# zhuker/lamejs

Measured on NVIDIA H100. Metric: encoded audio seconds/sec (44.1kHz stereo 128kbps CBR), higher is better.
Workload: dtype f64

## Files before the change

### lamejs_b200/csrc/k_quant.cuh

```cuda
#ifndef MP3B200_K_QUANT_CUH
#define MP3B200_K_QUANT_CUH
#include <stddef.h>
#include "mp3_device.cuh"
#include "mp3_tables.h"
#include "k_psy.cuh"

#define Q_LARGE_BITS 100000
#define Q_IXMAX 8206
#define Q_FULL 0xffffffffu

struct GranuleInfoDev {
  int global_gain, part2_3_length, part2_length, big_values, count1, scalefac_compress;
  int table_select[3], region0_count, region1_count, preflag, scalefac_scale, count1table_select, block_type;
  int subblock_gain[4];
  int count1bits, sfbmax, sfbdivide, sfb_lmax, psymax, psy_lmax, sfb_smin, max_nonzero_coeff;
  int scalefac[MP3_SFBMAX];
  int slen[4];
  int part_row;
  int pad_;
  double xrpow_max;
};
struct QuantFrameState {
  int stream, rel_frame;
  int in_old[2], in_step[2];
// ... 21 lines not shown
__device__ int g_t33l[16];
__constant__ int c_slen1_n[16];
__constant__ int c_slen2_n[16];
__device__ int g_slen_n[2][16];
__device__ int g_scale_tab[2][16];
__device__ unsigned int g_cat_tab[8][256];
__constant__ int c_slen1_tab[16];
__constant__ int c_slen2_tab[16];
__constant__ int c_huf_noesc[15];

static int quant_upload_constants() {
  static const int t32l[16] = {1, 5, 5, 7, 5, 8, 7, 9, 5, 7, 7, 9, 7, 9, 9, 10};
  static const int t33l[16] = {4, 5, 5, 6, 5, 6, 6, 7, 5, 6, 6, 7, 6, 7, 7, 8};
  static const int s1n[16] = {1, 1, 1, 1, 8, 2, 2, 2, 4, 4, 4, 8, 8, 8, 16, 16};
  static const int s2n[16] = {1, 2, 4, 8, 1, 2, 4, 8, 2, 4, 8, 2, 4, 8, 4, 8};
  static const int s1t[16] = {0, 0, 0, 0, 3, 1, 1, 1, 2, 2, 2, 3, 3, 3, 4, 4};
  static const int s2t[16] = {0, 1, 2, 3, 0, 1, 2, 3, 1, 2, 3, 1, 2, 3, 2, 3};
  static const int ss[16] = {0, 18, 36, 54, 54, 36, 54, 72, 54, 72, 90, 72, 90, 108, 108, 126};
  static const int sl[16] = {0, 10, 20, 30, 33, 21, 31, 41, 32, 42, 52, 43, 53, 63, 64, 74};
  static const int hn[15] = {1, 2, 5, 7, 7, 10, 10, 13, 13, 13, 13, 13, 13, 13, 13};
#define UP(sym, src) if (cudaMemcpyToSymbol(sym, src, sizeof(src)) != cudaSuccess) return -100
  UP(g_huff_code, MP3_HUFF_CODE); UP(g_huff_len, MP3_HUFF_LEN); UP(c_huff_off, MP3_HUFF_OFF);
  UP(c_huff_xlen, MP3_HUFF_XLEN);
  UP(g_t32l, t32l); UP(g_t33l, t33l); UP(c_slen1_n, s1n); UP(c_slen2_n, s2n);
  UP(c_slen1_tab, s1t); UP(c_slen2_tab, s2t); UP(c_huf_noesc, hn);
  {
    static int sn[2][16], st[2][16];
    static unsigned int ct[8][256];
    for (int k = 0; k < 16; k++) { sn[0][k] = s1n[k]; sn[1][k] = s2n[k]; st[0][k] = sl[k]; st[1][k] = ss[k]; }
    static const int fam[6] = {1, 2, 5, 7, 10, 13};
    for (int x = 0; x < 16; x++) for (int y = 0; y < 16; y++) {
      const int q = x * 16 + y;
      for (int c = 0; c < 6; c++) {
        const int t1 = fam[c], xl = MP3_HUFF_XLEN[t1];
        unsigned a = 0, b = 0, d = 0;
        if (x < xl && y < xl) {
          const int i = x * xl + y;
          if (c == 0) a = b = d = MP3_HUFF_LEN[MP3_HUFF_OFF[1] + i];
          else if (c == 1) { a = MP3_HUFF_TABLE23[i] >> 16; b = d = MP3_HUFF_TABLE23[i] & 0xffff; }
          else if (c == 2) { a = MP3_HUFF_TABLE56[i] >> 16; b = d = MP3_HUFF_TABLE56[i] & 0xffff; }
          else { a = MP3_HUFF_LEN[MP3_HUFF_OFF[t1] + i]; b = MP3_HUFF_LEN[MP3_HUFF_OFF[t1 + 1] + i]; d = MP3_HUFF_LEN[MP3_HUFF_OFF[t1 + 2] + i]; }
        }
        ct[c][q] = a | (b << 11) | (d << 22);
      }
      { const unsigned a = MP3_HUFF_LARGETBL[q] >> 16, b = MP3_HUFF_LARGETBL[q] & 0xffff; ct[6][q] = a | (b << 11) | (b << 22); }
      ct[7][q] = 0;
    }
    UP(g_slen_n, sn); UP(g_scale_tab, st); UP(g_cat_tab, ct);
  }
#undef UP
  return 0;
}

struct __align__(16) GcWork {
  float xrpow[576];
  short ixw[576];
  short* ixg;
  GranuleInfoDev w, b;
  const Mp3Geo* geo;
  float xmin[MP3_SFBMAX], distort[MP3_SFBMAX];
  int pn_step[MP3_SFBMAX]; float pn_noise[MP3_SFBMAX], pn_noise_log[MP3_SFBMAX];
  int pn_global_gain, pn_sfb_count1;
  unsigned char mode[MP3_SFBMAX + 1];
  short nstart[MP3_SFBMAX], nlen[MP3_SFBMAX];
  int scratch[8];
  double dscratch[4];
  __align__(16) float xr[576];
};
struct __align__(16) WarpShared {
  double ath[6];
  int scfsi[4];
  GcWork wk;
};
#define Q_STRIDE_NOXR ((int)((offsetof(WarpShared, wk) + offsetof(GcWork, xr) + 15) & ~(size_t)15))
static_assert((offsetof(WarpShared, wk) + offsetof(GcWork, xr)) % 16 == 0 && (offsetof(WarpShared, wk) + offsetof(GcWork, xrpow)) % 16 == 0 &&
              (offsetof(WarpShared, wk) + offsetof(GcWork, ixw)) % 16 == 0 && sizeof(WarpShared) % 16 == 0, "rows are moved as 16-byte vectors");
#ifndef Q_SLIM_BLOCKS
#define Q_SLIM_BLOCKS 9
#endif

#define LANE (threadIdx.x & 31)
#ifdef Q_TASKSTAT
__device__ int g_taskstat[1 << 16][8];
#endif
#ifdef Q_STATS
__device__ unsigned long long g_qstats[16];
#define QSTAT(i) do { if (LANE == 0) atomicAdd(&g_qstats[i], 1ull); } while (0)
#else
#define QSTAT(i) do { } while (0)
#endif
#define Q_PRAGMA(x) _Pragma(#x)
#define Q_UNROLL(n) Q_PRAGMA(unroll n)
#ifndef Q_RT_UNROLL
#define Q_RT_UNROLL 1
#endif
#ifndef Q_CB_UNROLL
#define Q_CB_UNROLL 1
#endif
#ifndef Q_CN_UNROLL
#define Q_CN_UNROLL 2
#endif
#ifndef Q_HELPER
#define Q_HELPER __forceinline__
#endif
#ifndef Q_SPEC_START
#define Q_SPEC_START 180
#endif
#ifndef Q_SPEC_STEP
#define Q_SPEC_STEP 32
#endif
#ifndef Q_SPEC_GR1_STEP
#define Q_SPEC_GR1_STEP 2
#endif
#ifndef Q_SPEC_FOLD
#define Q_SPEC_FOLD 1
#endif
#ifndef Q_MIN_BLOCKS
#define Q_MIN_BLOCKS 14
#endif
__device__ __noinline__ double q_log10(double x) { return m3_log10(x); }
__device__ __noinline__ double q_pow(double x, double y) { return m3_pow(x, y); }
__device__ __forceinline__ int wmax(int v) { return __reduce_max_sync(Q_FULL, v); }
__device__ __forceinline__ int wsum(int v) { return __reduce_add_sync(Q_FULL, v); }
__device__ __forceinline__ unsigned wsumu(unsigned v) { return __reduce_add_sync(Q_FULL, v); }

struct RegionClass { int cat; unsigned lin; int t1, t2; };
__device__ Q_HELPER RegionClass region_class(int mx) {
  RegionClass rc;
  rc.lin = 0; rc.t2 = 0;
  if (mx == 0) { rc.cat = 7; rc.t1 = 0; }
  else if (mx <= 15) {
    rc.t1 = c_huf_noesc[mx - 1];
    rc.cat = mx <= 3 ? mx - 1 : (mx <= 5 ? 3 : (mx <= 7 ? 4 : 5));
  } else {
    const int n = 32 - __clz(mx - 15);
    rc.t2 = 24 + (int)((0x7777665432100000ull >> (4 * n)) & 15ull);
    rc.t1 = max(rc.t2 - 8, 16 + (int)((0x7777766554432100ull >> (4 * n)) & 15ull));
    const unsigned la = (unsigned)c_huff_xlen[rc.t1], lb = (unsigned)c_huff_xlen[rc.t2];
    rc.lin = la | (lb << 11) | (lb << 22);
    rc.cat = 6;
  }
  return rc;
}
__device__ __forceinline__ unsigned pair_bits(unsigned w, int cat, unsigned lin) {
  const unsigned x = w & 0xffffu, y = w >> 16;
  const unsigned xe = min(x, 15u), ye = min(y, 15u);
  return __ldg(&g_cat_tab[cat][xe * 16 + ye]) + ((x > 14u) + (y > 14u)) * lin;
}
__device__ Q_HELPER int region_pick(int mx, const RegionClass& rc, int a, int b, int c, int* bits) {
  if (mx > Q_IXMAX) { *bits = Q_LARGE_BITS; return -1; }
  if (mx == 0) return 0;
  int t = rc.t1;
  if (mx <= 15) {
    if (a > b) { a = b; t++; }
    if (a > c) { a = c; t = rc.t1 + 2; }
  } else if (a > b) { a = b; t = rc.t2; }
  *bits += a;
  return t;
}

__device__ __noinline__ int region_table_w(const short* ix, int begin, int end, int* bits) {
  const int lane = LANE;
  const unsigned* w32 = reinterpret_cast<const unsigned*>(ix);
  const int p0 = (begin >> 1) + lane, p1 = end >> 1;
  unsigned m = 0;
Q_UNROLL(Q_RT_UNROLL)
// ... 275 lines not shown
  const bool is_short = gi->block_type == BT_SHORT;
  const int sfbmax = gi->sfbmax, sfbdivide = gi->sfbdivide;
  __syncwarp();
  if (!is_short && 0 == gi->preflag) {
    const bool in = lane >= 11 && lane < 21;
    const int pt = pretab_of(lane);
    const bool ok = !in || scalefac[lane] >= pt;
    if (__all_sync(Q_FULL, ok)) {
      __syncwarp();
      if (in) scalefac[lane] -= pt;
      if (lane == 0) gi->preflag = 1;
      __syncwarp();
    }
  }
  int m1 = 0, m2 = 0;
#pragma unroll 1
  for (int sfb = lane; sfb < sfbmax; sfb += 32) {
    const int v = scalefac[sfb];
    if (sfb < sfbdivide) m1 = max(m1, v); else m2 = max(m2, v);
  }
  m1 = wmax(m1); m2 = wmax(m2);
  int key = Q_LARGE_BITS * 16 + 15;
  if (lane < 16 && m1 < __ldg(&g_slen_n[0][lane]) && m2 < __ldg(&g_slen_n[1][lane])) key = __ldg(&g_scale_tab[is_short ? 1 : 0][lane]) * 16 + lane;
  key = __reduce_min_sync(Q_FULL, key);
  const int p2 = key >> 4;
  if (lane == 0) { gi->part2_length = p2; if (p2 != Q_LARGE_BITS) gi->scalefac_compress = key & 15; }
  __syncwarp();
  return p2 == Q_LARGE_BITS;
}

__device__ __noinline__ bool scale_bitcount_lsf_w(GranuleInfoDev* gi) {
  const int lane = LANE;
  const bool is_short = gi->block_type == BT_SHORT;
  __syncwarp();
  int m0 = 0, m1 = 0, m2 = 0, m3 = 0;
  const int n = is_short ? 36 : 21;
#pragma unroll 1
  for (int i = lane; i < n; i += 32) {
    const int v = gi->scalefac[i];
    const int p = is_short ? i / 9 : (i < 6 ? 0 : (i - 6) / 5 + 1);
    if (p == 0) m0 = max(m0, v); else if (p == 1) m1 = max(m1, v); else if (p == 2) m2 = max(m2, v); else m3 = max(m3, v);
  }
  m0 = wmax(m0); m1 = wmax(m1); m2 = wmax(m2); m3 = wmax(m3);
  const bool over = m0 > 15 || m1 > 15 || m2 > 7 || m3 > 7;
  if (!over && lane == 0) {
    const int s1 = m0 ? 32 - __clz(m0) : 0, s2 = m1 ? 32 - __clz(m1) : 0, s3 = m2 ? 32 - __clz(m2) : 0, s4 = m3 ? 32 - __clz(m3) : 0;
    gi->slen[0] = s1; gi->slen[1] = s2; gi->slen[2] = s3; gi->slen[3] = s4;
    gi->part_row = is_short ? 1 : 0;
    gi->scalefac_compress = (((s1 * 5) + s2) << 4) + (s3 << 2) + s4;
    gi->part2_length = is_short ? 9 * (s1 + s2 + s3 + s4) : 6 * s1 + 5 * (s2 + s3 + s4);
  }
  __syncwarp();
  return over;
}
__device__ __forceinline__ bool scale_bitcount_any_w(GranuleInfoDev* gi, int mode_gr) {
  return mode_gr == 2 ? scale_bitcount_w(gi) : scale_bitcount_lsf_w(gi);
}

__device__ __forceinline__ bool loop_break_w(const GranuleInfoDev* gi, const GcWork* wk) {
  bool nz = true;
#pragma unroll 1
  for (int sfb = LANE; sfb < gi->sfbmax; sfb += 32)
    if (gi->scalefac[sfb] + gi->subblock_gain[wk->geo->window[sfb]] == 0) nz = false;
  return __all_sync(Q_FULL, nz);
}

__device__ __noinline__ void scale_xrpow_w(GcWork* wk, GranuleInfoDev* gi, double f34) {
  const int lane = LANE;
  const int sfbmax = gi->sfbmax;
  float mx = 0.0f;
#pragma unroll 1
  for (int p = lane; p < 288; p += 32) {
    const int sfb = wk->geo->sfb_of_line[2 * p];
    if (sfb < sfbmax && wk->mode[sfb]) {
      float2* xp = reinterpret_cast<float2*>(&wk->xrpow[2 * p]);
      float2 x = *xp;
      f32s v0, v1; v0.v = x.x; v1.v = x.y;
      v0 *= f34; v1 *= f34;
      x.x = v0.v; x.y = v1.v;
      *xp = x;
      mx = fmaxf(mx, fmaxf(v0.v, v1.v));
    }
  }
#pragma unroll 1
  for (int o = 16; o > 0; o >>= 1) mx = fmaxf(mx, __shfl_xor_sync(Q_FULL, mx, o));
  if (lane == 0 && (double)mx > gi->xrpow_max) gi->xrpow_max = (double)mx;
  __syncwarp();
}

__device__ __noinline__ bool balance_escalate_w(const Mp3Tables* T, GcWork* wk) {
  const int lane = LANE;
  GranuleInfoDev* gi = &wk->w;
  int* flag = &wk->scratch[0];
  bool status = true;
  const int scale_now = gi->scalefac_scale, is_short_blk = gi->block_type == BT_SHORT;
  __syncwarp();
  if (T->noise_shaping > 1) {
    if (0 == scale_now) {
      {
        const int sfbmax = gi->sfbmax, pre = gi->preflag;
#pragma unroll 1
        for (int sfb = lane; sfb < sfbmax; sfb += 32) {
          int s = gi->scalefac[sfb];
          if (pre != 0) s += pretab_of(sfb);
          const int odd = (s & 1) != 0;
          if (odd) s++;
          wk->mode[sfb] = (unsigned char)odd;
          gi->scalefac[sfb] = s >> 1;
        }
        __syncwarp();
        if (lane == 0) { gi->preflag = 0; gi->scalefac_scale = 1; }
      }
      __syncwarp();
      scale_xrpow_w(wk, gi, 1.29683955465100964055);
      status = false;
    } else if (is_short_blk) {
      if (lane == 0) {
        int ret = 0;
        int* scalefac = gi->scalefac;
#pragma unroll 1
        for (int i = 0; i < MP3_SFBMAX; i++) wk->nlen[i] = -1;
#pragma unroll 1
        for (int window = 0; window < 3 && !ret; window++) {
          int s1 = 0, s2 = 0, sfb;
#pragma unroll 1
          for (sfb = gi->sfb_lmax + window; sfb < gi->sfbdivide; sfb += 3) if (s1 < scalefac[sfb]) s1 = scalefac[sfb];
#pragma unroll 1
          for (; sfb < gi->sfbmax; sfb += 3) if (s2 < scalefac[sfb]) s2 = scalefac[sfb];
          if (s1 < 16 && s2 < 8) continue;
          if (gi->subblock_gain[window] >= 7) { ret = 1; break; }
          gi->subblock_gain[window]++;
#pragma unroll 1
          for (sfb = gi->sfb_lmax + window; sfb < gi->sfbmax; sfb += 3) {
            int s = scalefac[sfb];
            s = s - (4 >> gi->scalefac_scale);
            if (s >= 0) { scalefac[sfb] = s; continue; }
            scalefac[sfb] = 0;
            wk->nlen[sfb] = 210 + s * (1 << (gi->scalefac_scale + 1));
          }
          wk->nlen[sfb] = 202;
        }
        *flag = ret;
      }
      __syncwarp();
      {
        float mx = 0.0f;
#pragma unroll 1
        for (int i = lane; i < 576; i += 32) {
          const int sfb = wk->geo->sfb_of_line[i];
          if (sfb < MP3_SFBMAX && wk->nlen[sfb] >= 0) {
            f32s v; v.v = wk->xrpow[i];
            v *= (double)T->ipow20[wk->nlen[sfb]];
            wk->xrpow[i] = v.v;
            mx = fmaxf(mx, v.v);
          }
        }
        for (int o = 16; o > 0; o >>= 1) mx = fmaxf(mx, __shfl_xor_sync(Q_FULL, mx, o));
        if (lane == 0 && (double)mx > gi->xrpow_max) gi->xrpow_max = (double)mx;
        __syncwarp();
      }
      {
        const int bailed = *flag;
        __syncwarp();
        status = bailed != 0 || loop_break_w(gi, wk);
      }
    }
  }
  if (!status) status = scale_bitcount_any_w(gi, T->mode_gr);
  return !status;
}


__device__ __noinline__ bool balance_noise_w(const Mp3Tables* T, GcWork* wk) {
  const int lane = LANE;
  GranuleInfoDev* gi = &wk->w;
  const double ifq = gi->scalefac_scale == 0 ? 1.29683955465100964055 : 1.68179283050742922612;
  {
    const int sfbmax = gi->sfbmax;
    double trigger = 0;
#pragma unroll 1
    for (int sfb = lane; sfb < sfbmax; sfb += 32) if (trigger < (double)wk->distort[sfb]) trigger = (double)wk->distort[sfb];
    for (int o = 16; o > 0; o >>= 1) { const double t = __shfl_xor_sync(Q_FULL, trigger, o); if (trigger < t) trigger = t; }
    if (trigger > 1.0) trigger = sqrt(trigger);
    else trigger *= .95;
#pragma unroll 1
    for (int sfb = lane; sfb < sfbmax; sfb += 32) {
      const int amp = !((double)wk->distort[sfb] < trigger);
      wk->mode[sfb] = (unsigned char)amp;
      if (amp) gi->scalefac[sfb]++;
    }
  }
  __syncwarp();
  scale_xrpow_w(wk, gi, ifq);
  int r;
  if (loop_break_w(gi, wk)) r = 0;
  else r = scale_bitcount_any_w(gi, T->mode_gr) ? 2 : 1;
  if (r == 0) return false;
  if (r == 1) return true;
  return balance_escalate_w(T, wk);
}

__device__ __noinline__ void copy_gi_w(GranuleInfoDev* dst, const GranuleInfoDev* src) {
  const int n = sizeof(GranuleInfoDev) / 4;
  const int* s = reinterpret_cast<const int*>(src);
  int* d = reinterpret_cast<int*>(dst);
  __syncwarp();
  static_assert(sizeof(GranuleInfoDev) / 4 <= 96, "three rounds");
  int v[3];
#pragma unroll
  for (int k = 0; k < 3; k++) { const int i = LANE + 32 * k; if (i < n) v[k] = s[i]; }
#pragma unroll
  for (int k = 0; k < 3; k++) { const int i = LANE + 32 * k; if (i < n) d[i] = v[k]; }
  __syncwarp();
}
__device__ __noinline__ void copy_ix_w(short* dst, const short* src) {
  const int* s = reinterpret_cast<const int*>(src);
  int* d = reinterpret_cast<int*>(dst);
  __syncwarp();
#pragma unroll 1
  for (int i = LANE; i < 288; i += 32) d[i] = s[i];
  __syncwarp();
}

__device__ __noinline__ int bin_search_w(const Mp3Tables* T, GcWork* wk, int desired_rate, int* old_value, int* current_step, int stat_base = 0) {
  GranuleInfoDev* gi = &wk->b;
  int nBits;
  int CurrentStep = *current_step;
  bool flagGoneOver = false;
  const int start = *old_value;
  int Direction = 0;
  int gain = start;
  desired_rate -= gi->part2_length;
  __syncwarp();
  for (;;) {
    int step;
    if (LANE == 0) gi->global_gain = gain;
    __syncwarp();
    QSTAT(stat_base);
    nBits = count_bits_w<false>(T, wk, gi, wk->ixw);
    if (CurrentStep == 1 || nBits == desired_rate) break;
    if (nBits > desired_rate) {
      if (Direction == 2) flagGoneOver = true;
      if (flagGoneOver) CurrentStep /= 2;
      Direction = 1;
      step = CurrentStep;
    } else {
      if (Direction == 1) flagGoneOver = true;
      if (flagGoneOver) CurrentStep /= 2;
      Direction = 2;
      step = -CurrentStep;
    }
    gain += step;
    if (gain < 0) { gain = 0; flagGoneOver = true; }
    if (gain > 255) { gain = 255; flagGoneOver = true; }
  }
  while (nBits > desired_rate && gain < 255) {
    gain++;
    if (LANE == 0) gi->global_gain = gain;
    __syncwarp();
    QSTAT(stat_base + 1);
    nBits = count_bits_w<false>(T, wk, gi, wk->ixw);
  }
  *current_step = (start - gain >= 4) ? 4 : 2;
  *old_value = gain;
  if (LANE == 0) gi->part2_3_length = nBits;
  __syncwarp();
  return nBits;
}

__device__ __noinline__ unsigned long long gi_hash(const GranuleInfoDev* gi) {
  const unsigned* w = reinterpret_cast<const unsigned*>(gi);
  unsigned sum = 0, x = 0;
#pragma unroll 1
  for (int i = LANE; i < (int)(sizeof(GranuleInfoDev) / 4); i += 32) {
    unsigned v = (w[i] ^ ((unsigned)i * 0x9E3779B9u)) * 0x85EBCA6Bu;
    v ^= v >> 13; v *= 0xC2B2AE35u; v ^= v >> 16;
    sum += v; x ^= __funnelshift_l(v, v, i & 31);
  }
  sum = __reduce_add_sync(Q_FULL, sum);
  x = __reduce_xor_sync(Q_FULL, x);
  return ((unsigned long long)sum << 32) | x;
}

__device__ __noinline__ void outer_loop_w(const Mp3Tables* T, GcWork* wk, int targ_bits) {
  const int lane = LANE;
  NoiseRes best, cur;
  int best_part2_3_length = 9999999;
#pragma unroll 1
  for (int i = lane; i < MP3_SFBMAX; i += 32) { wk->pn_step[i] = 0; wk->pn_noise[i] = 0.0f; wk->pn_noise_log[i] = 0.0f; }
  if (lane == 0) { wk->pn_global_gain = 0; wk->pn_sfb_count1 = 0; }
  __syncwarp();
  calc_noise_w(T, wk, &wk->b, wk->ixw, &best);
  best.bits = wk->b.part2_3_length;
  copy_gi_w(&wk->w, &wk->b);
  bool best_here = true;
  int age = 0;
  const int quant_comp = T->quant_comp;
  (void)quant_comp;
  do {
    const int search_limit = 3;
    int maxggain = 255;
    if (!balance_noise_w(T, wk)) break;
    GranuleInfoDev* w = &wk->w;
    if (w->scalefac_scale != 0) maxggain = 254;
    const int huff_bits = targ_bits - w->part2_length;
    if (huff_bits <= 0) break;
    int p23, gg;
    if (best_here) { copy_ix_w(wk->ixg, wk->ixw); best_here = false; }
    int sc_in;
    for (;;) {
      sc_in = wk->pn_sfb_count1;
      QSTAT(8);
      p23 = count_bits_w<true>(T, wk, w, wk->ixw);
      gg = w->global_gain;
      __syncwarp();
      if (!(p23 > huff_bits && gg <= maxggain)) break;
      if (lane == 0) w->global_gain = gg + 1;
      __syncwarp();
    }
    if (lane == 0) w->part2_3_length = p23;
    __syncwarp();
    if (gg > maxggain) break;
    if (best.over_count == 0) {
      bool repeat = wk->pn_sfb_count1 == sc_in;
      for (;;) {
        if (!repeat) { QSTAT(9); p23 = count_bits_w<true>(T, wk, w, wk->ixw); }
        repeat = false;
        gg = w->global_gain;
        __syncwarp();
        if (!(p23 > best_part2_3_length && gg <= maxggain)) break;
        if (lane == 0) w->global_gain = gg + 1;
        __syncwarp();
      }
      if (lane == 0) w->part2_3_length = p23;
      __syncwarp();
      if (gg > maxggain) break;
    }
    QSTAT(10);
    calc_noise_w(T, wk, w, wk->ixw, &cur);
    cur.bits = w->part2_3_length;
    bool better;
    if (best.over_count > 0) {
      better = cur.over_SSD <= best.over_SSD;
      if (cur.over_SSD == best.over_SSD) better = cur.bits < best.bits;
    } else {
      better = ((cur.max_noise < 0) && ((cur.max_noise * 10 + cur.bits) <= (best.max_noise * 10 + best.bits)));
    }
    if (best.over_count == 0) better = better && cur.bits < best.bits;
    if (better) {
      best_part2_3_length = wk->b.part2_3_length;
      best = cur;
      copy_gi_w(&wk->b, &wk->w);
      best_here = true;
      age = 0;
    } else {
      if (++age > search_limit && best.over_count == 0) break;
    }
    const int cont = (wk->w.global_gain + wk->w.scalefac_scale) < 255;
    __syncwarp();
    if (!cont) break;
  } while (true);
  if (!best_here) copy_ix_w(wk->ixw, wk->ixg);
}

__device__ __noinline__ double ath_adjust_dev(double a, double x, double athFloor) {
  const double o = 90.30873362, p = 94.82444863;
  double u = q_log10(x) * 10.0;
  const double v = a * a;
  double w = 0.0;
  u -= athFloor;
  if (v > 1E-20) w = 1. + q_log10(v) * (10.0 / o);
  if (w < 0) w = 0.;
  u *= w;
  u += athFloor + o - p;
  return q_pow(10., 0.1 * u);
}

__device__ __noinline__ bool gc_prepare_w(const Mp3Tables* T, GcWork* wk, const double* ath_ps, const float* __restrict__ xr_g, int block_type,
                             const PsyRatioDev* __restrict__ ratio, double ath_adjust) {
  const bool need_xmin = true;
  const int lane = LANE;
  GranuleInfoDev* gi = &wk->b;
  const bool is_short = block_type == BT_SHORT;
  if (lane == 0) {
    gi->part2_3_length = 0; gi->big_values = 0; gi->count1 = 0; gi->global_gain = 210; gi->scalefac_compress = 0;
    gi->table_select[0] = gi->table_select[1] = gi->table_select[2] = 0;
    gi->subblock_gain[0] = gi->subblock_gain[1] = gi->subblock_gain[2] = gi->subblock_gain[3] = 0;
    gi->region0_count = 0; gi->region1_count = 0; gi->preflag = 0; gi->scalefac_scale = 0; gi->count1table_select = 0;
    gi->part2_length = 0; gi->block_type = block_type; gi->count1bits = 0;
    gi->sfb_lmax = is_short ? 0 : 21; gi->sfb_smin = is_short ? 0 : 12;
    gi->psy_lmax = is_short ? 0 : 21;
    gi->psymax = is_short ? 36 : 21; gi->sfbmax = is_short ? 36 : 21; gi->sfbdivide = is_short ? 18 : 11;
    gi->max_nonzero_coeff = 575;
#pragma unroll 1
    for (int i = 0; i < MP3_SFBMAX; i++) gi->scalefac[i] = 0;
    gi->xrpow_max = 0;
  }
  const Mp3Geo* geo = &T->geo[is_short ? 1 : 0];
  if (lane == 0) wk->geo = geo;
  {
    float4 v[5];
#pragma unroll
    for (int k = 0; k < 5; k++) { const int q = lane + 32 * k; if (q < 144) v[k] = __ldg(reinterpret_cast<const float4*>(xr_g) + q); }
    if (!is_short) {
#pragma unroll
      for (int k = 0; k < 5; k++) { const int q = lane + 32 * k; if (q < 144) reinterpret_cast<float4*>(wk->xr)[q] = v[k]; }
    } else {
#pragma unroll
      for (int k = 0; k < 5; k++) {
        const int q = lane + 32 * k;
        if (q < 144) {
          const short* ro = geo->reorder + 4 * q;
          wk->xr[__ldg(ro + 0)] = v[k].x; wk->xr[__ldg(ro + 1)] = v[k].y; wk->xr[__ldg(ro + 2)] = v[k].z; wk->xr[__ldg(ro + 3)] = v[k].w;
        }
      }
    }
  }
  __syncwarp();
  if (!is_short) {
    const int lo = T->psfb21[0];
    const double lf = (double)T->longfact[21];
    int keep = lo - 1;
#pragma unroll 1
    for (int j = lo + lane; j < 576; j += 32) {
      int g = 0;
      while (g < 5 && j >= T->psfb21[g + 1]) g++;
      double ath21 = ath_ps[g];
      if (lf > 1e-12) ath21 *= lf;
      if (!(fabs((double)wk->xr[j]) < ath21)) keep = j;
    }
    keep = wmax(keep);
    __syncwarp();
#pragma unroll 1
    for (int j = keep + 1 + lane; j < 576; j += 32) wk->xr[j] = 0.0f;
  } else if (lane == 0) {
#pragma unroll 1
    for (int block = 0; block < 3; block++) {
      bool stop = false;
#pragma unroll 1
      for (int g = 5; g >= 0 && !stop; g--) {
        const int start = T->sfb_s[12] * 3 + (T->sfb_s[13] - T->sfb_s[12]) * block + (T->psfb12[g] - T->psfb12[0]);
        const int end = start + (T->psfb12[g + 1] - T->psfb12[g]);
        double ath12 = ath_ps[g];
        if ((double)T->shortfact[12] > 1e-12) ath12 *= (double)T->shortfact[12];
#pragma unroll 1
// ... 700 lines not shown
    int ov = gr == 0 ? q->in_old[ch] : q->bs_gain0[ch];
    int cs = gr == 0 ? q->in_step[ch] : q->bs_step0[ch];
    const GcPrep* pr = prep + gidx;
    const bool have = pr->have != 0;
    gi_init_w(&wk->b, pr);
    if (lane == 0) wk->geo = &T->geo[pr->block_type == BT_SHORT ? 1 : 0];
    unsigned long long h = 0;
    if (have) {
      copy_row16_w(wk->xrpow, xrpow_g + gidx * 576, 2304);
      QSTAT(revalidate ? 12 + gr : 11);
      bin_search_w(T, wk, targ, &ov, &cs, revalidate ? 2 + 2 * gr : 0);
      h = gi_hash(&wk->b);
    } else {
      __syncwarp();
#pragma unroll 1
      for (int i = lane; i < 288; i += 32) reinterpret_cast<unsigned*>(wk->ixw)[i] = 0;
      __syncwarp();
    }
    bool store;
    if (!revalidate) {
      store = true;
      if (gr == 0 && fg.f != 0 && T->mode_gr == 2) cs = Q_SPEC_GR1_STEP;
      if (lane == 0) {
        q->bs_hash[gr][ch] = h;
        if (gr == 0) { q->bs_gain0[ch] = ov; q->bs_step0[ch] = cs; }
        if (gr == T->mode_gr - 1) { q->out_old[ch] = ov; q->out_step[ch] = cs; }
      }
    } else if (gr == 0) {
      store = ov != q->bs_gain0[ch] || h != q->bs_hash[0][ch];
      const bool step_changed = cs != q->bs_step0[ch];
      __syncwarp();
      if (lane == 0) {
        int old = -1;
        if (T->mode_gr == 1) { q->out_old[ch] = ov; q->out_step[ch] = cs; }
        if (store) {
          q->bs_gain0[ch] = ov; q->bs_step0[ch] = cs; q->bs_hash[0][ch] = h; old = atomicOr(&q->redo, Q_R0(ch));
          if ((old & Q_R0_ANY) == 0) list3[atomicAdd(count3, 1)] = frow;
        } else if (step_changed && T->mode_gr == 2) { q->bs_step0[ch] = cs; old = atomicOr(&q->redo, Q_R1S(ch)); }
        if (old == 0) list2[atomicAdd(count2, 1)] = frow;
      }
    } else {
      store = (flags & Q_R0_ANY) || ov != q->out_old[ch] || h != q->bs_hash[1][ch];
      __syncwarp();
      if (lane == 0) {
        q->out_step[ch] = cs;
        if (store) { q->out_old[ch] = ov; q->bs_hash[1][ch] = h; atomicOr(&q->redo, Q_R1(ch)); }
      }
    }
    if (store) {
      copy_row16_w(l3enc + gidx * 576, wk->ixw, 1152);
      copy_gi_w(&ginfo[gidx], &wk->b);
    }
  }
}

__global__ void __launch_bounds__(Q_THREADS, Q_BLOCKS_PER_SM)
k_q_outer(const Mp3Tables* __restrict__ T, const StreamDesc* __restrict__ streams, QuantFrameState* __restrict__ qs,
          GranuleInfoDev* __restrict__ ginfo, short* __restrict__ l3enc, const float* __restrict__ xrq,
          const float* __restrict__ xrpow_g, const GcPrep* __restrict__ prep, int gr, const int* __restrict__ list,
          const int* __restrict__ count_ptr, int count_direct, int revalidate, int* __restrict__ counter) {
  WarpShared* ws = warp_shared();
  GcWork* wk = &ws->wk;
  const int lane = LANE, nch = T->nch;
  const int ntasks = (count_ptr ? *count_ptr : count_direct) * nch;
#pragma unroll 1
  for (int t = next_task(counter); t < ntasks; t = next_task(counter)) {
    const int wi = t / nch, ch = t - wi * nch;
#ifdef Q_REVERSE
    const int frow = list ? list[wi] : (ntasks / nch - 1 - wi);
#else
    const int frow = list ? list[wi] : wi;
#endif
    QuantFrameState* q = qs + frow;
    if (revalidate == 1 && !(q->redo & (gr == 0 ? Q_R0(ch) : Q_R1(ch)))) continue;
    if (revalidate == -1 && (q->redo & Q_R0_ANY)) continue;
    if (revalidate > 0) QSTAT(14);
    const FrameGeom fg = frame_geom(T, streams, q);
    const StreamDesc& sd = streams[fg.z];
    const size_t urow = (size_t)sd.unit_base + T->mode_gr * fg.f + gr, gidx = urow * nch + ch;
    const int targ = granule_budget(nch, fg.mean_bits, gr, q->used0[0], q->used0[1], ch);
    const GcPrep* pr = prep + gidx;
    const bool have = pr->have != 0;
    short* const ixrow = l3enc + gidx * 576;
    __syncwarp();
    if (lane == 0) { wk->geo = &T->geo[pr->block_type == BT_SHORT ? 1 : 0]; wk->ixg = ixrow; }
    copy_gi_w(&wk->b, &ginfo[gidx]);
    copy_row16_w(wk->ixw, ixrow, 1152);
#ifdef Q_TASKSTAT
    const long long ts_t0 = clock64();
    const int ts_gain = wk->b.global_gain, ts_bits = wk->b.part2_3_length;
#endif
    if (have) {
      copy_row16_w(wk->xr, xrq + gidx * 576, 2304);
      copy_row16_w(wk->xrpow, xrpow_g + gidx * 576, 2304);
#pragma unroll 1
      for (int i = lane; i < MP3_SFBMAX; i += 32) wk->xmin[i] = pr->xmin[i];
      __syncwarp();
      outer_loop_w(T, wk, targ);
    }
#ifdef Q_TASKSTAT
    if (lane == 0 && revalidate <= 0 && gidx < (1u << 16)) {
      int* r = g_taskstat[gidx];
      r[0] = (int)((clock64() - ts_t0) >> 6); r[1] = gr; r[2] = wk->b.max_nonzero_coeff; r[3] = wk->b.block_type;
      r[4] = ts_gain; r[5] = ts_bits; r[6] = targ; r[7] = wk->b.global_gain;
    }
#endif
    copy_gi_w(&ginfo[gidx], &wk->b);
    copy_row16_w(ixrow, wk->ixw, 1152);
  }
}

__global__ void __launch_bounds__(Q_THREADS, Q_SLIM_BLOCKS)
k_q_finish(const Mp3Tables* __restrict__ T, const StreamDesc* __restrict__ streams, QuantFrameState* __restrict__ qs,
           GranuleInfoDev* __restrict__ ginfo, short* __restrict__ l3enc, int gr, const int* __restrict__ list,
           const int* __restrict__ count_ptr, int count_direct, int revalidate, int* __restrict__ counter) {
  WarpShared* ws = warp_shared<Q_STRIDE_NOXR>();
  GcWork* wk = &ws->wk;
  const int lane = LANE, nch = T->nch;
  const int ntasks = (count_ptr ? *count_ptr : count_direct) * nch;
#pragma unroll 1
  for (int t = next_task(counter); t < ntasks; t = next_task(counter)) {
    const int wi = t / nch, ch = t - wi * nch;
    const int frow = list ? list[wi] : wi;
    QuantFrameState* q = qs + frow;
    if (revalidate == 1 && !(q->redo & (gr == 0 ? Q_R0(ch) : Q_R1(ch)))) continue;
    if (revalidate == -1 && (q->redo & Q_R0_ANY)) continue;
    const StreamDesc& sd = streams[q->stream];
    const size_t urow = (size_t)sd.unit_base + T->mode_gr * q->rel_frame + gr, gidx = urow * nch + ch;
    short* const ixrow = l3enc + gidx * 576;
    copy_gi_w(&wk->b, &ginfo[gidx]);
    copy_row16_w(wk->ixw, ixrow, 1152);
    if (lane == 0) wk->geo = &T->geo[wk->b.block_type == BT_SHORT ? 1 : 0];
    __syncwarp();
    best_scalefac_store_w(wk, ws->scfsi, gr == 1 ? &ginfo[gidx - nch] : nullptr, gr, T->mode_gr);
    best_huffman_divide_w(T, wk);
    copy_gi_w(&ginfo[gidx], &wk->b);
    if (gr == 0) { if (lane == 0) q->used0[ch] = wk->b.part2_3_length + wk->b.part2_length; }
    else if (lane < 4) q->scfsi[ch][lane] = ws->scfsi[lane];
  }
}

struct __align__(16) PackShared {
  unsigned int bits[368];
  short ix[576];
  unsigned neg[20];
  GranuleInfoDev gi;
  int scfsi[8];
};
__global__ void __launch_bounds__(Q_THREADS)
k_q_pack(const Mp3Tables* __restrict__ T, const StreamDesc* __restrict__ streams, QuantFrameState* __restrict__ qs,
         const GranuleInfoDev* __restrict__ ginfo, const short* __restrict__ l3enc, const unsigned* __restrict__ neg_g,
         const int* __restrict__ list, const int* __restrict__ count_ptr, int count_direct, int revalidate,
         int* __restrict__ counter, uint8_t* __restrict__ out) {
  extern __shared__ __align__(16) unsigned char smem_raw[];
  PackShared* ps = reinterpret_cast<PackShared*>(smem_raw) + (threadIdx.x >> 5);
  const int lane = LANE, nch = T->nch;
  const int ntasks = count_ptr ? *count_ptr : count_direct;
#pragma unroll 1
  for (int t = next_task(counter); t < ntasks; t = next_task(counter)) {
    const int frow = list ? list[t] : t;
    QuantFrameState* q = qs + frow;
    if (revalidate && !(q->redo & (Q_R0_ANY | Q_R1_ANY))) continue;
    if (revalidate) QSTAT(5);
    const FrameGeom fg = frame_geom(T, streams, q);
    const StreamDesc& sd = streams[fg.z];
    const size_t g0 = ((size_t)sd.unit_base + T->mode_gr * fg.f) * nch;
    __syncwarp();
#pragma unroll 1
    for (int i = lane; i < 368; i += 32) ps->bits[i] = 0;
    if (lane < 8) ps->scfsi[lane] = q->scfsi[lane >> 2][lane & 3];
    __syncwarp();
    int pos = 8 * T->sideinfo_len;
#pragma unroll 1
    for (int k = 0; k < T->mode_gr * nch; k++) {
      copy_gi_w(&ps->gi, &ginfo[g0 + k]);
      copy_row16_w(ps->ix, l3enc + (g0 + k) * 576, 1152);
      if (lane < 18) ps->neg[lane] = neg_g[(g0 + k) * 18 + lane];
      __syncwarp();
      pack_gc_w(T, ps->bits, &ps->gi, ps->ix, ps->neg, pos);
      pos += ps->gi.part2_3_length + ps->gi.part2_length;
      __syncwarp();
    }
    if (lane == 0) {
      pack_sideinfo(T, ps->bits, ginfo + g0, ps->scfsi, fg.padding);
      int remaining = 8 * fg.frame_bytes - pos;
      const unsigned char tag[10] = {0x4c, 0x41, 0x4d, 0x45, 3, 0, 9, 8, 0, 4};
      int k = 0;
      for (; k < 4 && remaining >= 8; k++) { put_bits(ps->bits, pos, tag[k], 8); pos += 8; remaining -= 8; }
      if (remaining >= 32) for (; k < 10 && remaining >= 8; k++) { put_bits(ps->bits, pos, tag[k], 8); pos += 8; remaining -= 8; }
    }
    __syncwarp();
// ... 217 lines not shown
```

### lamejs_b200/csrc/mp3_encoder.cu

```cuda
#include <cuda_runtime.h>
#include <stdio.h>
#include <stdlib.h>
#include <string.h>
#include <atomic>
#include <map>
#include <mutex>
#include <string>
#include <tuple>
#include <vector>

#include "../../include/mp3b200.h"
#include "mp3_config.h"
#include "mp3_device.cuh"
#include "mp3_tables.h"
#include "k_filterbank.cuh"
#include "k_psy.cuh"
#include "k_quant.cuh"
#include "k_tag.cuh"
#include "mp3_tag.h"

namespace {

thread_local std::string g_err;
std::mutex g_mu;
// ... 736 lines not shown
                          uint8_t* buf, int cap) {
  Mp3TagParams p;
  if (mp3_tag_params(channels, samplerate, kbps, &p) != 0) { g_err = "unsupported configuration"; return MP3B200_ERR_CONFIG; }
  if (!p.fits || nframes <= 0) return 0;
  if (!buf || cap < p.frame_bytes) return p.frame_bytes;
  Mp3SeekBag* bag = new Mp3SeekBag();
  bag->reset();
  bag->add_frames(nframes, p.kbps);
  const int n = mp3_tag_frame(p, *bag, music_bytes, (unsigned)music_crc, encoder_padding, buf);
  delete bag;
  return n;
}

int mp3b200_encode_streams_tagged(int channels, int samplerate, int kbps, int nstreams, const int16_t* const* left,
                                  const int16_t* const* right, const int64_t* nsamples, uint8_t* const* out,
                                  const int64_t* cap, int64_t* out_bytes) {
  if (nstreams < 0) { g_err = "negative stream count"; return MP3B200_ERR_HANDLE; }
  Config* cfg;
  int rc = get_config(channels, samplerate, kbps, &cfg);
  if (rc) return rc;
  Mp3TagParams p;
  if (mp3_tag_params(channels, samplerate, kbps, &p) != 0) { g_err = "unsupported configuration"; return MP3B200_ERR_CONFIG; }
  const int tfs = p.fits ? p.frame_bytes : 0;
  std::vector<int64_t> pcm_off(nstreams), out_off(nstreams);
  std::vector<long long> frames(nstreams), audio(nstreams);
  long long tot_samples = 0, tot_bytes = 0;
  for (int s = 0; s < nstreams; s++) {
    pcm_off[s] = tot_samples; tot_samples += nsamples[s] * channels;
    out_off[s] = tot_bytes;
    frames[s] = frames_for(nsamples[s], cfg->host.mode_gr);
    audio[s] = bytes_for(cfg->host, frames[s]);
    if (cap[s] < audio[s] + tfs) { g_err = "output buffer too small"; return MP3B200_ERR_BUFFER; }
    out_bytes[s] = audio[s] + tfs;
    tot_bytes += audio[s];
  }
  if (nstreams == 0) return MP3B200_OK;
  rc = t_ctx.use(cfg->device);
  if (rc) return rc;
  rc = t_ctx.need_pcm((size_t)tot_samples + 8);
  if (rc) return rc;
  rc = t_ctx.need_out((size_t)tot_bytes + 8);
  if (rc) return rc;
  for (int s = 0; s < nstreams; s++) {
    if (nsamples[s] <= 0) continue;
    CK(cudaMemcpyAsync(t_ctx.d_pcm + pcm_off[s], left[s], sizeof(int16_t) * nsamples[s], cudaMemcpyHostToDevice, t_ctx.up_st));
    if (channels == 2)
      CK(cudaMemcpyAsync(t_ctx.d_pcm + pcm_off[s] + nsamples[s], (right && right[s]) ? right[s] : left[s], sizeof(int16_t) * nsamples[s], cudaMemcpyHostToDevice, t_ctx.up_st));
  }
  PcmArrival arr;
  arr.chunks = 1; arr.ready = t_ctx.ready;
  CK(cudaEventRecord(t_ctx.ready[0], t_ctx.up_st));
  rc = encode_streams_device_impl(cfg, channels, nstreams, t_ctx.d_pcm, pcm_off.data(), nsamples, t_ctx.d_out, out_off.data(), nullptr, &arr);
  if (rc) return rc;
  std::vector<long long> off(out_off.begin(), out_off.end());
  std::vector<unsigned> crc;
  rc = music_crc_ranges(cfg->device, t_ctx.d_out, off, audio, crc);
  if (rc) return rc;
  Mp3SeekBag* bag = new Mp3SeekBag();
  for (int s = 0; s < nstreams; s++) {
    int wrote = 0;
    if (tfs > 0 && frames[s] > 0) {
      bag->reset();
      bag->add_frames(frames[s], p.kbps);
      wrote = mp3_tag_frame(p, *bag, audio[s], crc[s], mp3_encoder_padding(nsamples[s], cfg->host.mode_gr), out[s]);
    }
    out_bytes[s] = audio[s] + wrote;
    if (audio[s] > 0 && cudaMemcpyAsync(out[s] + wrote, t_ctx.d_out + out_off[s], (size_t)audio[s], cudaMemcpyDeviceToHost, t_ctx.st) != cudaSuccess) rc = MP3B200_ERR_CUDA;
  }
  delete bag;
  if (cudaStreamSynchronize(t_ctx.st) != cudaSuccess) rc = MP3B200_ERR_CUDA;
  return rc;
}

}

#include "mp3_handle.inc"

#ifdef Q_TASKSTAT
extern "C" int mp3b200_debug_taskstat(int* out, int rows) {
  if (rows > (1 << 16)) rows = 1 << 16;
  return cudaMemcpyFromSymbol(out, g_taskstat, sizeof(int) * 8 * (size_t)rows) == cudaSuccess ? 0 : -1;
}
#endif
```

Measured before the change: 51120.

## Fuse balance_noise loops into register-resident warp reductions and add phase profiling

Rewrites balance_noise_w so each lane holds up to two scalefactor bands in registers. It computes the trigger with an integer __reduce_max_sync on the float bits, and folds the loop_break check, the preflag decision and the MPEG-1 scale_bitcount into a few warp reductions (__reduce_and/min_sync) instead of separate noinline passes over shared memory. scale_xrpow_w's shuffle reduction is replaced with __reduce_max_sync. It also adds opt-in Q_PHASESTAT clock64 instrumentation, compiled out by default. The change assumes sfbmax is at most 64 and non-negative distortions, which the inline bitcount must match exactly to keep output identical.

```diff
diff --git a/lamejs_b200/csrc/k_quant.cuh b/lamejs_b200/csrc/k_quant.cuh
--- a/lamejs_b200/csrc/k_quant.cuh
+++ b/lamejs_b200/csrc/k_quant.cuh
@@ -127,6 +127,20 @@
 #define LANE (threadIdx.x & 31)
 #ifdef Q_TASKSTAT
 __device__ int g_taskstat[1 << 16][8];
+#endif
+#ifdef Q_PHASESTAT
+enum { QP_BALANCE, QP_GAIN1, QP_GAIN2, QP_NOISE, QP_COMPARE, QP_ROWS, QP_TOTAL, QP_GR };
+__device__ long long g_phasestat[1 << 16][8];
+__device__ long long g_phase_acc[1 << 14][6];
+#define QP_PARAM , long long* qp_acc
+#define QP_ARG , qp_acc
+#define QP_BEGIN(v) const long long v = clock64()
+#define QP_END(v, ph) do { if (LANE == 0) qp_acc[ph] += clock64() - (v); } while (0)
+#else
+#define QP_PARAM
+#define QP_ARG
+#define QP_BEGIN(v) do { } while (0)
+#define QP_END(v, ph) do { } while (0)
 #endif
 #ifdef Q_STATS
 __device__ unsigned long long g_qstats[16];
@@ -568,8 +582,7 @@
       mx = fmaxf(mx, fmaxf(v0.v, v1.v));
     }
   }
-#pragma unroll 1
-  for (int o = 16; o > 0; o >>= 1) mx = fmaxf(mx, __shfl_xor_sync(Q_FULL, mx, o));
+  mx = __int_as_float(__reduce_max_sync(Q_FULL, __float_as_int(mx)));
   if (lane == 0 && (double)mx > gi->xrpow_max) gi->xrpow_max = (double)mx;
   __syncwarp();
 }
@@ -661,28 +674,60 @@
   const int lane = LANE;
   GranuleInfoDev* gi = &wk->w;
   const double ifq = gi->scalefac_scale == 0 ? 1.29683955465100964055 : 1.68179283050742922612;
-  {
-    const int sfbmax = gi->sfbmax;
-    double trigger = 0;
-#pragma unroll 1
-    for (int sfb = lane; sfb < sfbmax; sfb += 32) if (trigger < (double)wk->distort[sfb]) trigger = (double)wk->distort[sfb];
-    for (int o = 16; o > 0; o >>= 1) { const double t = __shfl_xor_sync(Q_FULL, trigger, o); if (trigger < t) trigger = t; }
-    if (trigger > 1.0) trigger = sqrt(trigger);
-    else trigger *= .95;
-#pragma unroll 1
-    for (int sfb = lane; sfb < sfbmax; sfb += 32) {
-      const int amp = !((double)wk->distort[sfb] < trigger);
-      wk->mode[sfb] = (unsigned char)amp;
-      if (amp) gi->scalefac[sfb]++;
-    }
+  const int sfbmax = gi->sfbmax, s1 = lane + 32;
+  const bool h0 = lane < sfbmax, h1 = s1 < sfbmax;
+  const float d0 = h0 ? wk->distort[lane] : 0.0f, d1 = h1 ? wk->distort[s1] : 0.0f;
+  double trigger = (double)__int_as_float(__reduce_max_sync(Q_FULL, max(d0 > 0.0f ? __float_as_int(d0) : 0, d1 > 0.0f ? __float_as_int(d1) : 0)));
+  if (trigger > 1.0) trigger = sqrt(trigger);
+  else trigger *= .95;
+  int sf0 = 0, sf1 = 0;
+  bool nz = true;
+  if (h0) {
+    const int amp = !((double)d0 < trigger);
+    sf0 = gi->scalefac[lane] + amp;
+    wk->mode[lane] = (unsigned char)amp;
+    if (amp) gi->scalefac[lane] = sf0;
+    nz = sf0 + gi->subblock_gain[wk->geo->window[lane]] != 0;
+  }
+  if (h1) {
+    const int amp = !((double)d1 < trigger);
+    sf1 = gi->scalefac[s1] + amp;
+    wk->mode[s1] = (unsigned char)amp;
+    if (amp) gi->scalefac[s1] = sf1;
+    nz = nz && sf1 + gi->subblock_gain[wk->geo->window[s1]] != 0;
   }
   __syncwarp();
   scale_xrpow_w(wk, gi, ifq);
-  int r;
-  if (loop_break_w(gi, wk)) r = 0;
-  else r = scale_bitcount_any_w(gi, T->mode_gr) ? 2 : 1;
-  if (r == 0) return false;
-  if (r == 1) return true;
+  const bool mpeg1 = T->mode_gr == 2;
+  const bool pf_in = lane >= 11 && lane < 21;
+  const int pt = pretab_of(lane);
+  const unsigned ok = __reduce_and_sync(Q_FULL, (nz ? 1u : 0u) | ((!pf_in || sf0 >= pt) ? 2u : 0u));
+  if (ok & 1u) return false;
+  bool over;
+  if (mpeg1) {
+    const bool is_short = gi->block_type == BT_SHORT;
+    if (!is_short && 0 == gi->preflag && (ok & 2u)) {
+      __syncwarp();
+      if (pf_in) { sf0 -= pt; gi->scalefac[lane] = sf0; }
+      if (lane == 0) gi->preflag = 1;
+    }
+    const int sfbdivide = gi->sfbdivide;
+    int m1 = 0, m2 = 0;
+    if (h0) { if (lane < sfbdivide) m1 = sf0; else m2 = sf0; }
+    if (h1) { if (s1 < sfbdivide) m1 = max(m1, sf1); else m2 = max(m2, sf1); }
+    m1 = wmax(m1); m2 = wmax(m2);
+    int key = Q_LARGE_BITS * 16 + 15;
+    if (lane < 16 && m1 < __ldg(&g_slen_n[0][lane]) && m2 < __ldg(&g_slen_n[1][lane])) key = __ldg(&g_scale_tab[is_short ? 1 : 0][lane]) * 16 + lane;
+    key = __reduce_min_sync(Q_FULL, key);
+    const int p2 = key >> 4;
+    __syncwarp();
+    if (lane == 0) { gi->part2_length = p2; if (p2 != Q_LARGE_BITS) gi->scalefac_compress = key & 15; }
+    __syncwarp();
+    over = p2 == Q_LARGE_BITS;
+  } else {
+    over = scale_bitcount_lsf_w(gi);
+  }
+  if (!over) return true;
   return balance_escalate_w(T, wk);
 }
 
@@ -768,7 +813,7 @@
   return ((unsigned long long)sum << 32) | x;
 }
 
-__device__ __noinline__ void outer_loop_w(const Mp3Tables* T, GcWork* wk, int targ_bits) {
+__device__ __noinline__ void outer_loop_w(const Mp3Tables* T, GcWork* wk, int targ_bits QP_PARAM) {
   const int lane = LANE;
   NoiseRes best, cur;
   int best_part2_3_length = 9999999;
@@ -776,9 +821,13 @@
   for (int i = lane; i < MP3_SFBMAX; i += 32) { wk->pn_step[i] = 0; wk->pn_noise[i] = 0.0f; wk->pn_noise_log[i] = 0.0f; }
   if (lane == 0) { wk->pn_global_gain = 0; wk->pn_sfb_count1 = 0; }
   __syncwarp();
+  QP_BEGIN(qp_n0);
   calc_noise_w(T, wk, &wk->b, wk->ixw, &best);
+  QP_END(qp_n0, QP_NOISE);
+  QP_BEGIN(qp_c0);
   best.bits = wk->b.part2_3_length;
   copy_gi_w(&wk->w, &wk->b);
+  QP_END(qp_c0, QP_COMPARE);
   bool best_here = true;
   int age = 0;
   const int quant_comp = T->quant_comp;
@@ -786,13 +835,19 @@
   do {
     const int search_limit = 3;
     int maxggain = 255;
-    if (!balance_noise_w(T, wk)) break;
+    QP_BEGIN(qp_b);
+    const bool bal = balance_noise_w(T, wk);
+    QP_END(qp_b, QP_BALANCE);
+    if (!bal) break;
     GranuleInfoDev* w = &wk->w;
     if (w->scalefac_scale != 0) maxggain = 254;
     const int huff_bits = targ_bits - w->part2_length;
     if (huff_bits <= 0) break;
     int p23, gg;
+    QP_BEGIN(qp_p);
     if (best_here) { copy_ix_w(wk->ixg, wk->ixw); best_here = false; }
+    QP_END(qp_p, QP_COMPARE);
+    QP_BEGIN(qp_g1);
     int sc_in;
     for (;;) {
       sc_in = wk->pn_sfb_count1;
@@ -806,8 +861,10 @@
     }
     if (lane == 0) w->part2_3_length = p23;
     __syncwarp();
+    QP_END(qp_g1, QP_GAIN1);
     if (gg > maxggain) break;
     if (best.over_count == 0) {
+      QP_BEGIN(qp_g2);
       bool repeat = wk->pn_sfb_count1 == sc_in;
       for (;;) {
         if (!repeat) { QSTAT(9); p23 = count_bits_w<true>(T, wk, w, wk->ixw); }
@@ -820,10 +877,14 @@
       }
       if (lane == 0) w->part2_3_length = p23;
       __syncwarp();
+      QP_END(qp_g2, QP_GAIN2);
       if (gg > maxggain) break;
     }
     QSTAT(10);
+    QP_BEGIN(qp_n);
     calc_noise_w(T, wk, w, wk->ixw, &cur);
+    QP_END(qp_n, QP_NOISE);
+    QP_BEGIN(qp_c);
     cur.bits = w->part2_3_length;
     bool better;
     if (best.over_count > 0) {
@@ -840,13 +901,16 @@
       best_here = true;
       age = 0;
     } else {
-      if (++age > search_limit && best.over_count == 0) break;
+      if (++age > search_limit && best.over_count == 0) { QP_END(qp_c, QP_COMPARE); break; }
     }
     const int cont = (wk->w.global_gain + wk->w.scalefac_scale) < 255;
     __syncwarp();
+    QP_END(qp_c, QP_COMPARE);
     if (!cont) break;
   } while (true);
+  QP_BEGIN(qp_e);
   if (!best_here) copy_ix_w(wk->ixw, wk->ixg);
+  QP_END(qp_e, QP_COMPARE);
 }
 
 __device__ __noinline__ double ath_adjust_dev(double a, double x, double athFloor) {
@@ -1713,6 +1777,13 @@
     const GcPrep* pr = prep + gidx;
     const bool have = pr->have != 0;
     short* const ixrow = l3enc + gidx * 576;
+#ifdef Q_PHASESTAT
+    long long* const qp_acc = g_phase_acc[(revalidate > 0 ? 1 << 13 : 0) + blockIdx.x * Q_WARPS + (threadIdx.x >> 5)];
+    if (lane < 6) qp_acc[lane] = 0;
+    __syncwarp();
+#endif
+    QP_BEGIN(qp_task);
+    QP_BEGIN(qp_ld);
     __syncwarp();
     if (lane == 0) { wk->geo = &T->geo[pr->block_type == BT_SHORT ? 1 : 0]; wk->ixg = ixrow; }
     copy_gi_w(&wk->b, &ginfo[gidx]);
@@ -1727,8 +1798,12 @@
 #pragma unroll 1
       for (int i = lane; i < MP3_SFBMAX; i += 32) wk->xmin[i] = pr->xmin[i];
       __syncwarp();
-      outer_loop_w(T, wk, targ);
-    }
+      QP_END(qp_ld, QP_ROWS);
+      outer_loop_w(T, wk, targ QP_ARG);
+    }
+#ifdef Q_PHASESTAT
+    else QP_END(qp_ld, QP_ROWS);
+#endif
 #ifdef Q_TASKSTAT
     if (lane == 0 && revalidate <= 0 && gidx < (1u << 16)) {
       int* r = g_taskstat[gidx];
@@ -1736,8 +1811,17 @@
       r[4] = ts_gain; r[5] = ts_bits; r[6] = targ; r[7] = wk->b.global_gain;
     }
 #endif
+    QP_BEGIN(qp_st);
     copy_gi_w(&ginfo[gidx], &wk->b);
     copy_row16_w(ixrow, wk->ixw, 1152);
+    QP_END(qp_st, QP_ROWS);
+#ifdef Q_PHASESTAT
+    if (lane == 0 && revalidate <= 0 && gidx < (1u << 16)) {
+      long long* r = g_phasestat[gidx];
+      for (int k = 0; k < 6; k++) r[k] = qp_acc[k];
+      r[QP_TOTAL] = clock64() - qp_task; r[QP_GR] = gr;
+    }
+#endif
   }
 }
 
diff --git a/lamejs_b200/csrc/mp3_encoder.cu b/lamejs_b200/csrc/mp3_encoder.cu
--- a/lamejs_b200/csrc/mp3_encoder.cu
+++ b/lamejs_b200/csrc/mp3_encoder.cu
@@ -842,3 +842,9 @@
   return cudaMemcpyFromSymbol(out, g_taskstat, sizeof(int) * 8 * (size_t)rows) == cudaSuccess ? 0 : -1;
 }
 #endif
+#ifdef Q_PHASESTAT
+extern "C" int mp3b200_debug_phasestat(long long* out, int rows) {
+  if (rows > (1 << 16)) rows = 1 << 16;
+  return cudaMemcpyFromSymbol(out, g_phasestat, sizeof(long long) * 8 * (size_t)rows) == cudaSuccess ? 0 : -1;
+}
+#endif
```

Result: faster. 52960, median of 6 (+3.6%).
